# Runki2018/litehandnet

Measured on AMD Instinct MI355X. Metric: images/sec fwd+bwd @256x256 bs64 litehandnet, higher is better.
Workload: dtype f32; 1 GPU; litehandnet variant B (MSRB hourglass litehourglass.py) C=128, 256x256x3 -> 21x64x64, per-GPU batch 64, train-mode BN, fwd + TopdownHeatmapLoss + bwd + fused Adam; global_batch=64, parallelism=dp1

## Files before the change

### litehandnet_amd/csrc/k_conv_dw.hip

```cpp
#include <stdlib.h>
#include "lhn_common.h"

template <int K>
__global__ void __launch_bounds__(256) k_dw_fwd(lhn_view x, const float* __restrict__ w, lhn_view y,
                                                double* __restrict__ stats, int stride, int pad, int dil, lhn_bnfin fin,
                                                int ) {
  extern __shared__ __attribute__((aligned(16))) float smem[];
  const int C = x.C, C4 = C >> 2;
  constexpr int KK = K * K;
  float* Ws = smem;
  f4* red = reinterpret_cast<f4*>(smem + KK * C);
  const int tid = threadIdx.x;
  const int c4 = tid % C4, pl = tid / C4, PL = 256 / C4;
  const int cin = x.coff + 4 * c4, cout = y.coff + 4 * c4;
  const Xf4 xf = lhn_load_xf(x, cin);
  for (int i = tid; i < KK * C; i += 256) {
    const int c = i / KK, t = i - c * KK;
    Ws[t * C + c] = w ? w[i] : 1.f;
  }
  __syncthreads();
  f4 wt[KK];
#pragma unroll
  for (int t = 0; t < KK; ++t) wt[t] = *reinterpret_cast<const f4*>(Ws + t * C + 4 * c4);
  const int rows = y.N * y.H;
// ... 1064 lines not shown
        const int ih = h0 + ph, iw = w0 + pw;
        const bool inb = ih >= 0 && ih < SH && iw >= 0 && iw < SW;
        f4 v = lhn_apply_xf(raw[it], xf) * gate;
        if (NS > 1) {
          v += lhn_apply_xf(raw2[it], xf2) * gate2;
          if (ex.sum_out && cok && inb && ph >= T::P && ph < T::P + TH && pw >= T::P && pw < T::P + TW)
            *reinterpret_cast<f4*>(ex.sum_out + ((size_t)(n * x.H + pa + ps * ih) * x.W + pb + ps * iw) * ex.so_cstride + ex.so_coff +
                                   cg * 32 + 4 * c4) = v;
        }
        tile[i * 8 + c4] = inb ? v : (f4){0.f, 0.f, 0.f, 0.f};
      }
    }
    __syncthreads();
    if (t + (int)gridDim.x < ntile) issue(t + gridDim.x);
    const int wo = tw * TW + pl;
    f4 s = (f4){0.f, 0.f, 0.f, 0.f}, q = s, kk = s;
    int cnt = 0;
    if (wo < SW && cok) {
      const f4* col = tile + (pl + T::P) * 8 + c4;
      float* yout = y.data + ((size_t)(n * y.H + pa + ps * th * TH) * y.W + pb + ps * wo) * y.cstride + cout;
      if (K == 3 && DIL == 1) {
        f4 wt[9];
#pragma unroll
        for (int k = 0; k < 9; ++k) wt[k] = wl[k * 8 + c4];
        f4 win[3][3];
#pragma unroll
        for (int a = 0; a < 2; ++a)
#pragma unroll
          for (int b = 0; b < 3; ++b) win[a + 1][b] = col[(a * T::WW + (b - 1)) * 8];
#pragma unroll
        for (int rr = 0; rr < TH; ++rr) {
#pragma unroll
          for (int b = 0; b < 3; ++b) {
            win[0][b] = win[1][b];
            win[1][b] = win[2][b];
            win[2][b] = col[((rr + 2) * T::WW + (b - 1)) * 8];
          }
          if (th * TH + rr < SH) {
            f4 acc = (f4){0.f, 0.f, 0.f, 0.f};
#pragma unroll
            for (int a = 0; a < 3; ++a)
#pragma unroll
              for (int b = 0; b < 3; ++b) acc += win[a][b] * wt[a * 3 + b];
            *reinterpret_cast<f4*>(yout + (size_t)rr * ps * y.W * y.cstride) = acc;
            if (cnt == 0) kk = acc;
            const f4 d = acc - kk;
            s += d;
            q += d * d;
            ++cnt;
          }
        }
      } else {
        for (int rr = 0; rr < TH; ++rr) {
          if (th * TH + rr >= SH) break;
          f4 acc = (f4){0.f, 0.f, 0.f, 0.f};
#pragma unroll
          for (int a = 0; a < K; ++a)
#pragma unroll
            for (int b = 0; b < K; ++b)
              acc += col[((rr + a * DIL) * T::WW + (b * DIL - T::P)) * 8] * wl[(a * K + b) * 8 + c4];
          *reinterpret_cast<f4*>(yout + (size_t)rr * ps * y.W * y.cstride) = acc;
          if (cnt == 0) kk = acc;
          const f4 d = acc - kk;
          s += d;
          q += d * d;
          ++cnt;
        }
      }
    }
    lhn_unshift4(sd, qd, s, q, kk, cnt);
  }
  if (stats) {
    const int C = x.C;
    double* st = stats + (size_t)((bid / cgroups) % LHN_STAT_REPLICAS) * 2 * C + cg * 32;
    lhn_block_stat_atomics_d(sd, qd, 8, reinterpret_cast<double*>(red), st, st + C, cvalid);
    if (fin.counter && lhn_last_block(fin.counter)) lhn_bn_finalize_block_par(fin, stats, reinterpret_cast<double*>(red));
  }
}

struct DwBnSum {
  double* sums;
  const float* save;
  int C, coff;
  const float* add[2];
};

template <int K, int DIL, bool BNS = false>
__global__ void __launch_bounds__(256) k_dwk_bwd_lds(lhn_view x, const float* __restrict__ w, lhn_view y, lhn_gradview gy,
                                                     float* __restrict__ dx, int dx_acc, float* __restrict__ dw, int tiles_h,
                                                     int tiles_w, int cgroups, int nrep, int64_t rep_stride, int ps, DwBnSum bs, int xchunk) {
  constexpr int TH = 8, TW = 16, KK = K * K;
  const int bid = xchunk ? (int)(blockIdx.x & 7) * xchunk + (int)(blockIdx.x >> 3) : (int)blockIdx.x;
  constexpr bool REGACC = (K == 3);
  using T = DwTile<K, DIL, TH, TW>;
  extern __shared__ __attribute__((aligned(16))) float smem[];
  f4* tdy = reinterpret_cast<f4*>(smem);
  f4* tx = tdy + T::PIX * 8;
  f4* red = tx + T::PIX * 8;
  f4* wl = red + 256;
  f4* dws = wl + KK * 8;
  f4* traw = dws + KK * 8;
  f4* tmi = traw + TH * TW * 8;
  const int tid = threadIdx.x, c4 = tid & 7, pl = tid >> 3;
  const int colw = pl & 15, rpar = pl >> 4;
  const int ntile = y.N * ps * ps * tiles_h * tiles_w * cgroups;
  const int cg = bid % cgroups;
  const int cvalid = min(8, (x.C - cg * 32) >> 2);
  const bool cok = c4 < cvalid;
  const int c4e = cok ? c4 : 0;
  const int cx = x.coff + cg * 32 + 4 * c4e, cy = y.coff + cg * 32 + 4 * c4e;
  const Xf4 xxf = lhn_load_xf(x, cx), yxf = lhn_load_xf(y, cy);
  const Gr4 ygr = lhn_load_coef(gy, y.cstride, cy);
  for (int i = tid; i < KK * 8; i += 256) {
    const int k = i >> 3, cc = cg * 32 + 4 * min(i & 7, cvalid - 1);
    wl[i] = (f4){w[(cc + 0) * KK + k], w[(cc + 1) * KK + k], w[(cc + 2) * KK + k], w[(cc + 3) * KK + k]};
    if (!REGACC) dws[i] = (f4){0.f, 0.f, 0.f, 0.f};
  }
  f4 accw[REGACC ? KK : 1];
#pragma unroll
  for (int k = 0; k < (REGACC ? KK : 1); ++k) accw[k] = (f4){0.f, 0.f, 0.f, 0.f};
  f4 sdu = (f4){0.f, 0.f, 0.f, 0.f}, sdux = sdu;
  if (BNS && tid < 16) {
    const int kind = tid >> 3, cc = tid & 7;
    tmi[tid] = *reinterpret_cast<const f4*>(bs.save + kind * bs.C + bs.coff + cg * 32 + 4 * cc);
  }
  for (int t = bid; t < ntile; t += gridDim.x) {
    int r = t / cgroups;
    const int tw = r % tiles_w;
    r /= tiles_w;
    const int th = r % tiles_h;
    r /= tiles_h;
    const int par = r % (ps * ps), n = r / (ps * ps), pa = par / ps, pb = par % ps;
    const int SH = (x.H - pa + ps - 1) / ps, SW = (x.W - pb + ps - 1) / ps;
    const f4 xgate = x.gate ? *reinterpret_cast<const f4*>(x.gate + (size_t)n * x.cstride + cx) : (f4){1.f, 1.f, 1.f, 1.f};
    const f4 ygate = y.gate ? *reinterpret_cast<const f4*>(y.gate + (size_t)n * y.cstride + cy) : (f4){1.f, 1.f, 1.f, 1.f};
    const int h0 = th * TH - T::P, w0 = tw * TW - T::P;
    __syncthreads();
    {
      constexpr int NIT = (T::PIX + 31) / 32;
      f4 rx[NIT], ry[NIT], rz[NIT];
#pragma unroll
      for (int it = 0; it < NIT; ++it) {
        const int i = min(pl + 32 * it, T::PIX - 1);
        const int ph = i / T::WW, pw = i - ph * T::WW;
        const int ih = min(pa + ps * min(max(h0 + ph, 0), max(SH - 1, 0)), x.H - 1);
        const int iw = min(pb + ps * min(max(w0 + pw, 0), max(SW - 1, 0)), x.W - 1);
        const size_t pix = (size_t)(n * x.H + ih) * x.W + iw;
        rx[it] = *reinterpret_cast<const f4*>(x.data + pix * x.cstride + cx);
        ry[it] = *reinterpret_cast<const f4*>(y.data + pix * y.cstride + cy);
        rz[it] = *reinterpret_cast<const f4*>(gy.dz + pix * y.cstride + cy);
      }
#pragma unroll
      for (int it = 0; it < NIT; ++it) {
        const int i = pl + 32 * it;
        if (i < T::PIX) {
          const int ph = i / T::WW, pw = i - ph * T::WW;
          const int ih = h0 + ph, iw = w0 + pw;
          const bool inb = ih >= 0 && ih < SH && iw >= 0 && iw < SW;
          const f4 vx = lhn_apply_xf(rx[it], xxf) * xgate;
          f4 e = rz[it] * ygate;
          const f4 u = ry[it] * yxf.sc + yxf.sh;
          const f4 dl = (f4){u.x > 0.f ? 1.f : yxf.sl.x, u.y > 0.f ? 1.f : yxf.sl.y, u.z > 0.f ? 1.f : yxf.sl.z,
                             u.w > 0.f ? 1.f : yxf.sl.w};
          if (gy.dpool && inb) e += lhn_dpool_sum(gy, y, n, pa + ps * ih, pb + ps * iw, cy);
          const f4 vy = ygr.A * (e * dl) + ygr.B * ry[it] + ygr.Cc;
          const f4 z = (f4){0.f, 0.f, 0.f, 0.f};
          tx[i * 8 + c4] = inb ? vx : z;
          tdy[i * 8 + c4] = inb ? vy : z;
          if (BNS && ph >= T::P && ph < T::P + TH && pw >= T::P && pw < T::P + TW) traw[((ph - T::P) * TW + pw - T::P) * 8 + c4] = rx[it];
        }
      }
    }
    __syncthreads();
    const int wcol = tw * TW + colw;
    if (REGACC) {
#pragma unroll
      for (int j = 0; j < TH / 2; ++j) {
        const int rr = 2 * j + rpar, hh = th * TH + rr;
        if (wcol < SW && hh < SH) {
          const int centre = ((rr + T::P) * T::WW + colw + T::P) * 8 + c4;
          const f4 dyc = tdy[centre];
          f4 accx = (f4){0.f, 0.f, 0.f, 0.f};
#pragma unroll
          for (int a = 0; a < K; ++a)
#pragma unroll
            for (int b = 0; b < K; ++b) {
              const int off = ((a * DIL - T::P) * T::WW + (b * DIL - T::P)) * 8;
              accx += tdy[centre - off] * wl[(a * K + b) * 8 + c4];
              accw[REGACC ? a * K + b : 0] += dyc * tx[centre + off];
            }
          if (BNS) {
            const f4 raw = traw[(rr * TW + colw) * 8 + c4];
            const f4 u = raw * xxf.sc + xxf.sh;
            const f4 du = accx * (f4){u.x > 0.f ? 1.f : xxf.sl.x, u.y > 0.f ? 1.f : xxf.sl.y, u.z > 0.f ? 1.f : xxf.sl.z, u.w > 0.f ? 1.f : xxf.sl.w};
            sdu += du;
            sdux += du * ((raw - tmi[c4]) * tmi[8 + c4]);
          }
          if (dx && cok) {
            float* o = dx + ((size_t)(n * x.H + pa + ps * hh) * x.W + pb + ps * wcol) * x.cstride + cx;
            if (dx_acc) accx += *reinterpret_cast<const f4*>(o);
            if (bs.add[0]) accx += *reinterpret_cast<const f4*>(bs.add[0] + (o - dx));
            if (bs.add[1]) accx += *reinterpret_cast<const f4*>(bs.add[1] + (o - dx));
            *reinterpret_cast<f4*>(o) = accx;
          }
        }
      }
    } else {
      if (dx)
        for (int j = 0; j < TH / 2; ++j) {
          const int rr = 2 * j + rpar, hh = th * TH + rr;
          if (wcol < SW && hh < SH && cok) {
            const int centre = ((rr + T::P) * T::WW + colw + T::P) * 8 + c4;
            f4 accx = (f4){0.f, 0.f, 0.f, 0.f};
            for (int a = 0; a < K; ++a)
#pragma unroll
              for (int b = 0; b < K; ++b)
                accx += tdy[centre - ((a * DIL - T::P) * T::WW + (b * DIL - T::P)) * 8] * wl[(a * K + b) * 8 + c4];
            float* o = dx + ((size_t)(n * x.H + pa + ps * hh) * x.W + pb + ps * wcol) * x.cstride + cx;
            if (dx_acc) accx += *reinterpret_cast<const f4*>(o);
            if (bs.add[0]) accx += *reinterpret_cast<const f4*>(bs.add[0] + (o - dx));
            if (bs.add[1]) accx += *reinterpret_cast<const f4*>(bs.add[1] + (o - dx));
            *reinterpret_cast<f4*>(o) = accx;
          }
        }
      for (int a = 0; a < K; ++a) {
        f4 ar[K];
#pragma unroll
        for (int b = 0; b < K; ++b) ar[b] = (f4){0.f, 0.f, 0.f, 0.f};
        for (int j = 0; j < TH / 2; ++j) {
          const int rr = 2 * j + rpar, hh = th * TH + rr;
          if (wcol < SW && hh < SH) {
            const int centre = ((rr + T::P) * T::WW + colw + T::P) * 8 + c4;
            const f4 dyc = tdy[centre];
#pragma unroll
            for (int b = 0; b < K; ++b) ar[b] += dyc * tx[centre + ((a * DIL - T::P) * T::WW + (b * DIL - T::P)) * 8];
          }
        }
#pragma unroll
        for (int b = 0; b < K; ++b) {
          f4 v = ar[b];
#pragma unroll
          for (int o = 8; o < 64; o <<= 1) {
            v.x += __shfl_xor(v.x, o, 64);
            v.y += __shfl_xor(v.y, o, 64);
            v.z += __shfl_xor(v.z, o, 64);
            v.w += __shfl_xor(v.w, o, 64);
          }
          if ((tid & 63) < 8) red[(tid >> 6) * 8 + c4 + 32 * b] = v;
        }
        __syncthreads();
        if (tid < 8 * K) {
          const int b = tid >> 3, cc = tid & 7;
          dws[(a * K + b) * 8 + cc] += red[cc + 32 * b] + red[8 + cc + 32 * b] + red[16 + cc + 32 * b] + red[24 + cc + 32 * b];
        }
        __syncthreads();
      }
    }
  }
  if (BNS) {
    double* st = bs.sums + (size_t)((bid / cgroups) % LHN_STAT_REPLICAS) * 2 * bs.C + bs.coff + cg * 32;
    lhn_block_stat_atomics(sdu, sdux, 8, red, st, st + bs.C);
  }
  float* dwr = dw + (size_t)((bid / cgroups) % nrep) * rep_stride;
  if (REGACC) {
#pragma unroll
    for (int k = 0; k < KK; ++k)
#pragma unroll
      for (int o = 8; o < 64; o <<= 1) {
        accw[k].x += __shfl_xor(accw[k].x, o, 64);
        accw[k].y += __shfl_xor(accw[k].y, o, 64);
        accw[k].z += __shfl_xor(accw[k].z, o, 64);
        accw[k].w += __shfl_xor(accw[k].w, o, 64);
      }
    __syncthreads();
    if ((tid & 63) < 8)
#pragma unroll
      for (int k = 0; k < KK; ++k) tdy[(k * 4 + (tid >> 6)) * 8 + c4] = accw[k];
    __syncthreads();
    if (tid < KK * 8) {
      const int k = tid >> 3, cc = tid & 7;
      const f4 sacc = tdy[(k * 4 + 0) * 8 + cc] + tdy[(k * 4 + 1) * 8 + cc] + tdy[(k * 4 + 2) * 8 + cc] + tdy[(k * 4 + 3) * 8 + cc];
      const int cb = cg * 32 + 4 * cc;
      if (cc < cvalid) {
        atomicAdd(dwr + (cb + 0) * KK + k, sacc.x);
        atomicAdd(dwr + (cb + 1) * KK + k, sacc.y);
        atomicAdd(dwr + (cb + 2) * KK + k, sacc.z);
        atomicAdd(dwr + (cb + 3) * KK + k, sacc.w);
      }
    }
  } else {
    __syncthreads();
    for (int i = tid; i < KK * 8; i += 256) {
      const int k = i >> 3, cb = cg * 32 + 4 * (i & 7);
      const f4 v = dws[i];
      if ((i & 7) >= cvalid) continue;
      atomicAdd(dwr + (cb + 0) * KK + k, v.x);
      atomicAdd(dwr + (cb + 1) * KK + k, v.y);
      atomicAdd(dwr + (cb + 2) * KK + k, v.z);
      atomicAdd(dwr + (cb + 3) * KK + k, v.w);
    }
  }
}

static int dw3_xchunk(int grid, int cgroups) {
  static int on = -1;
  if (on < 0) {
    const char* e = getenv("LHN_XCD_ORDER");
    on = (e && e[0] == '1') ? 1 : 0;
  }
  return (on && grid % (8 * cgroups) == 0) ? grid / 8 : 0;
}
static int dw3_grid(int ntile, int cgroups, int per_cu) {
  int g = lhn_num_cus() * per_cu;
  g -= g % cgroups;
  if (g > ntile) g = ntile;
  if (g < cgroups) g = cgroups;
  return g;
}

template <int K, int DIL, int NS = 1>
static void launch_dwk_fwd(const lhn_view* x, const float* w, const lhn_view* y, double* stats, lhn_bnfin fin, hipStream_t s, int ps = 1,
                           const DwExtra* exp = nullptr) {
  DwExtra ex;
  if (exp) ex = *exp; else { ex.n = 0; ex.sum_out = nullptr; }
  constexpr int TH = 8, TW = 32, P = DIL * (K - 1) / 2;
  const int cg = (x->C + 31) / 32;
  const int sh = (y->H + ps - 1) / ps, sw = (y->W + ps - 1) / ps;
  const int th = (sh + TH - 1) / TH, tw = (sw + TW - 1) / TW, ntile = y->N * ps * ps * th * tw * cg;
  const size_t lds = (size_t)((TH + 2 * P) * (TW + 2 * P) * 8 + 512 + K * K * 8) * 16;
  const int per_cu = lds > 80 * 1024 ? 1 : (lds > 52 * 1024 ? 2 : 3);
  static LhnKernelCfg cfg;
  (void)lhn_kernel_cfg(cfg, &k_dwk_fwd_lds<K, DIL, NS>, lds, 4, nullptr);
  const int grid = dw3_grid(ntile, cg, per_cu * 2);
  hipLaunchKernelGGL((k_dwk_fwd_lds<K, DIL, NS>), dim3(grid), dim3(256), lds, s, *x, w, *y, stats, th, tw, cg, fin, ps, ex, dw3_xchunk(grid, cg));
}
template <int K, int DIL, bool BNS = false>
static void launch_dwk_bwd(const lhn_view* x, const float* w, const lhn_view* y, const lhn_gradview* gy, float* dx, int dx_acc,
                           float* dw, int nrep, int64_t rep_stride, hipStream_t s, int ps = 1, const DwBnSum* bsp = nullptr) {
  constexpr int TH = 8, TW = 16, P = DIL * (K - 1) / 2;
  DwBnSum bs;
  if (bsp) bs = *bsp; else { bs.sums = nullptr; bs.save = nullptr; bs.C = bs.coff = 0; bs.add[0] = bs.add[1] = nullptr; }
  const int cg = (x->C + 31) / 32;
  const int sh = (x->H + ps - 1) / ps, sw = (x->W + ps - 1) / ps;
  const int th = (sh + TH - 1) / TH, tw = (sw + TW - 1) / TW, ntile = x->N * ps * ps * th * tw * cg;
  const size_t lds = (size_t)((TH + 2 * P) * (TW + 2 * P) * 16 + 256 + 2 * K * K * 8 + (BNS ? TH * TW * 8 + 16 : 0)) * 16;
  static LhnKernelCfg cfg;
  (void)lhn_kernel_cfg(cfg, &k_dwk_bwd_lds<K, DIL, BNS>, lds, 4, nullptr);
  const int grid = dw3_grid(ntile, cg, 4);
  hipLaunchKernelGGL((k_dwk_bwd_lds<K, DIL, BNS>), dim3(grid), dim3(256), lds, s, *x, w, *y, *gy, dx, dx_acc, dw, th, tw,
                     cg, nrep, rep_stride, ps, bs, dw3_xchunk(grid, cg));
}


struct DwS2 {
  static constexpr int TH = 4, TW = 16, XH = 2 * TH + 1, XW = 2 * TW + 1, XPIX = XH * XW, DH = TH + 1, DW = TW + 1, DPIX = DH * DW;
};

__global__ void __launch_bounds__(256) k_dws2_fwd_lds(lhn_view x, const float* __restrict__ w, lhn_view y, double* __restrict__ stats,
                                                      int tiles_h, int tiles_w, int cgroups, lhn_bnfin fin) {
  using T = DwS2;
  extern __shared__ __attribute__((aligned(16))) float smem[];
  f4* tx = reinterpret_cast<f4*>(smem);
  f4* red = tx + T::XPIX * 8;
  f4* wl = red + 512;
  const int tid = threadIdx.x, c4 = tid & 7, pl = tid >> 3;
  const int ntile = y.N * tiles_h * tiles_w * cgroups;
  const int cg = blockIdx.x % cgroups;
  const int cvalid = min(8, (x.C - cg * 32) >> 2);
  const bool cok = c4 < cvalid;
  const int c4e = cok ? c4 : 0;
  const int cin = x.coff + cg * 32 + 4 * c4e, cout = y.coff + cg * 32 + 4 * c4e;
  for (int i = tid; i < 72; i += 256) {
    const int k = i >> 3, cc = cg * 32 + 4 * min(i & 7, cvalid - 1);
    wl[i] = (f4){w[(cc + 0) * 9 + k], w[(cc + 1) * 9 + k], w[(cc + 2) * 9 + k], w[(cc + 3) * 9 + k]};
  }
  const Xf4 xf = lhn_load_xf(x, cin);
  double sd[4] = {0, 0, 0, 0}, qd[4] = {0, 0, 0, 0};
  constexpr int NIT = (T::XPIX + 31) / 32;
  for (int t = blockIdx.x; t < ntile; t += gridDim.x) {
    int r = t / cgroups;
    const int tw = r % tiles_w;
    r /= tiles_w;
    const int th = r % tiles_h, n = r / tiles_h;
    const int h0 = 2 * th * T::TH - 1, w0 = 2 * tw * T::TW - 1;
    const f4 gate = x.gate ? *reinterpret_cast<const f4*>(x.gate + (size_t)n * x.cstride + cin) : (f4){1.f, 1.f, 1.f, 1.f};
    const float* xin = x.data + (size_t)n * x.H * x.W * x.cstride + cin;
    f4 raw[NIT];
#pragma unroll
    for (int it = 0; it < NIT; ++it) {
      const int i = min(pl + 32 * it, T::XPIX - 1);
      const int ph = i / T::XW, pw = i - ph * T::XW;
      const int ih = min(max(h0 + ph, 0), x.H - 1), iw = min(max(w0 + pw, 0), x.W - 1);
      raw[it] = *reinterpret_cast<const f4*>(xin + ((size_t)ih * x.W + iw) * x.cstride);
    }
    __syncthreads();
#pragma unroll
    for (int it = 0; it < NIT; ++it) {
      const int i = pl + 32 * it;
      if (i < T::XPIX) {
        const int ph = i / T::XW, pw = i - ph * T::XW;
        const int ih = h0 + ph, iw = w0 + pw;
        const bool inb = ih >= 0 && ih < x.H && iw >= 0 && iw < x.W;
        tx[i * 8 + c4] = inb ? lhn_apply_xf(raw[it], xf) * gate : (f4){0.f, 0.f, 0.f, 0.f};
      }
    }
    __syncthreads();
    f4 s = (f4){0.f, 0.f, 0.f, 0.f}, q = s, kk = s;
    int cnt = 0;
#pragma unroll
    for (int j = 0; j < 2; ++j) {
      const int o = pl + 32 * j, oh = o / T::TW, ow = o - oh * T::TW;
      const int ho = th * T::TH + oh, wo = tw * T::TW + ow;
      if (cok && ho < y.H && wo < y.W) {
        f4 acc = (f4){0.f, 0.f, 0.f, 0.f};
#pragma unroll
        for (int a = 0; a < 3; ++a)
#pragma unroll
          for (int b = 0; b < 3; ++b) acc += tx[((2 * oh + a) * T::XW + 2 * ow + b) * 8 + c4] * wl[(a * 3 + b) * 8 + c4];
        *reinterpret_cast<f4*>(y.data + ((size_t)(n * y.H + ho) * y.W + wo) * y.cstride + cout) = acc;
        if (cnt == 0) kk = acc;
        const f4 d = acc - kk;
        s += d;
        q += d * d;
        ++cnt;
      }
    }
    lhn_unshift4(sd, qd, s, q, kk, cnt);
  }
  if (stats) {
    const int C = x.C;
    double* st = stats + (size_t)((blockIdx.x / cgroups) % LHN_STAT_REPLICAS) * 2 * C + cg * 32;
    lhn_block_stat_atomics_d(sd, qd, 8, reinterpret_cast<double*>(red), st, st + C, cvalid);
    if (fin.counter && lhn_last_block(fin.counter)) lhn_bn_finalize_block(fin, stats);
  }
}

__global__ void __launch_bounds__(256, 2) k_dws2_bwd_lds(lhn_view x, const float* __restrict__ w, lhn_view y, lhn_gradview gy,
                                                      float* __restrict__ dx, int dx_acc, float* __restrict__ dw, int tiles_h,
                                                      int tiles_w, int cgroups, int nrep, int64_t rep_stride) {
  using T = DwS2;
  extern __shared__ __attribute__((aligned(16))) float smem[];
  f4* tx = reinterpret_cast<f4*>(smem);
  f4* tdy = tx + T::XPIX * 8;
  f4* wl = tdy + T::DPIX * 8;
  const int tid = threadIdx.x, c4 = tid & 7, pl = tid >> 3;
  const int ntile = y.N * tiles_h * tiles_w * cgroups;
  const int cg = blockIdx.x % cgroups;
  const int cvalid = min(8, (x.C - cg * 32) >> 2);
  const bool cok = c4 < cvalid;
  const int c4e = cok ? c4 : 0;
  const int cx = x.coff + cg * 32 + 4 * c4e, cy = y.coff + cg * 32 + 4 * c4e;
  const Xf4 xxf = lhn_load_xf(x, cx), yxf = lhn_load_xf(y, cy);
  const Gr4 ygr = lhn_load_coef(gy, y.cstride, cy);
  for (int i = tid; i < 72; i += 256) {
    const int k = i >> 3, cc = cg * 32 + 4 * min(i & 7, cvalid - 1);
    wl[i] = (f4){w[(cc + 0) * 9 + k], w[(cc + 1) * 9 + k], w[(cc + 2) * 9 + k], w[(cc + 3) * 9 + k]};
  }
  f4 accw[9];
#pragma unroll
  for (int k = 0; k < 9; ++k) accw[k] = (f4){0.f, 0.f, 0.f, 0.f};
  constexpr int NITX = (T::XPIX + 31) / 32, NITD = (T::DPIX + 31) / 32;
  for (int t = blockIdx.x; t < ntile; t += gridDim.x) {
    int r = t / cgroups;
    const int tw = r % tiles_w;
    r /= tiles_w;
    const int th = r % tiles_h, n = r / tiles_h;
    const int h0 = 2 * th * T::TH - 1, w0 = 2 * tw * T::TW - 1;
    const int oh0 = th * T::TH, ow0 = tw * T::TW;
    const f4 xgate = x.gate ? *reinterpret_cast<const f4*>(x.gate + (size_t)n * x.cstride + cx) : (f4){1.f, 1.f, 1.f, 1.f};
    f4 rx[NITX], ry[NITD], rz[NITD];
#pragma unroll
    for (int it = 0; it < NITX; ++it) {
      const int i = min(pl + 32 * it, T::XPIX - 1);
      const int ph = i / T::XW, pw = i - ph * T::XW;
      const int ih = min(max(h0 + ph, 0), x.H - 1), iw = min(max(w0 + pw, 0), x.W - 1);
      rx[it] = *reinterpret_cast<const f4*>(x.data + ((size_t)(n * x.H + ih) * x.W + iw) * x.cstride + cx);
    }
#pragma unroll
    for (int it = 0; it < NITD; ++it) {
      const int i = min(pl + 32 * it, T::DPIX - 1);
      const int ph = i / T::DW, pw = i - ph * T::DW;
      const int ho = min(oh0 + ph, y.H - 1), wo = min(ow0 + pw, y.W - 1);
      const size_t off = ((size_t)(n * y.H + ho) * y.W + wo) * y.cstride + cy;
      ry[it] = *reinterpret_cast<const f4*>(y.data + off);
      rz[it] = *reinterpret_cast<const f4*>(gy.dz + off);
    }
    __syncthreads();
#pragma unroll
    for (int it = 0; it < NITX; ++it) {
      const int i = pl + 32 * it;
      if (i < T::XPIX) {
        const int ph = i / T::XW, pw = i - ph * T::XW;
        const int ih = h0 + ph, iw = w0 + pw;
        const bool inb = ih >= 0 && ih < x.H && iw >= 0 && iw < x.W;
        tx[i * 8 + c4] = inb ? lhn_apply_xf(rx[it], xxf) * xgate : (f4){0.f, 0.f, 0.f, 0.f};
      }
    }
#pragma unroll
    for (int it = 0; it < NITD; ++it) {
      const int i = pl + 32 * it;
      if (i < T::DPIX) {
        const int ph = i / T::DW, pw = i - ph * T::DW;
        const int ho = oh0 + ph, wo = ow0 + pw;
        f4 d = (f4){0.f, 0.f, 0.f, 0.f};
        if (ho < y.H && wo < y.W) {
          const f4 du = lhn_grad_du(y, gy, yxf, ry[it], rz[it], n, ho, wo, cy);
          d = ygr.A * du + ygr.B * ry[it] + ygr.Cc;
        }
        tdy[i * 8 + c4] = d;
      }
    }
    __syncthreads();
#pragma unroll
    for (int j = 0; j < 2; ++j) {
      const int o = pl + 32 * j, oh = o / T::TW, ow = o - oh * T::TW;
      const f4 dyc = tdy[(oh * T::DW + ow) * 8 + c4];
#pragma unroll
      for (int a = 0; a < 3; ++a)
#pragma unroll
        for (int b = 0; b < 3; ++b) accw[a * 3 + b] += dyc * tx[((2 * oh + a) * T::XW + 2 * ow + b) * 8 + c4];
    }
    if (dx && cok) {
      const int c = pl, iw = 2 * ow0 + c;
      const int nb = (c & 1) ? 2 : 1;
      const int bA = (c & 1) ? 0 : 1, colA = (c & 1) ? (c + 1) >> 1 : c >> 1, colB = (c - 1) >> 1;
      if (iw < x.W) {
#pragma unroll
        for (int rr = 0; rr < 2 * T::TH; ++rr) {
          const int ih = 2 * oh0 + rr;
          if (ih < x.H) {
            f4 accx = (f4){0.f, 0.f, 0.f, 0.f};
            if ((rr & 1) == 0) {
              const f4* drow = tdy + ((rr >> 1) * T::DW) * 8 + c4;
              accx += drow[colA * 8] * wl[(3 + bA) * 8 + c4];
              if (nb == 2) accx += drow[colB * 8] * wl[(3 + 2) * 8 + c4];
            } else {
              const f4* d0 = tdy + (((rr + 1) >> 1) * T::DW) * 8 + c4;
              const f4* d2 = tdy + (((rr - 1) >> 1) * T::DW) * 8 + c4;
              accx += d0[colA * 8] * wl[(0 + bA) * 8 + c4] + d2[colA * 8] * wl[(6 + bA) * 8 + c4];
              if (nb == 2) accx += d0[colB * 8] * wl[(0 + 2) * 8 + c4] + d2[colB * 8] * wl[(6 + 2) * 8 + c4];
            }
            float* o = dx + ((size_t)(n * x.H + ih) * x.W + iw) * x.cstride + cx;
            if (dx_acc) accx += *reinterpret_cast<const f4*>(o);
            *reinterpret_cast<f4*>(o) = accx;
          }
        }
      }
    }
  }
  float* dwr = dw + (size_t)((blockIdx.x / cgroups) % nrep) * rep_stride;
#pragma unroll
  for (int k = 0; k < 9; ++k)
#pragma unroll
    for (int o = 8; o < 64; o <<= 1) {
      accw[k].x += __shfl_xor(accw[k].x, o, 64);
      accw[k].y += __shfl_xor(accw[k].y, o, 64);
      accw[k].z += __shfl_xor(accw[k].z, o, 64);
      accw[k].w += __shfl_xor(accw[k].w, o, 64);
    }
  __syncthreads();
  if ((tid & 63) < 8)
#pragma unroll
    for (int k = 0; k < 9; ++k) tdy[(k * 4 + (tid >> 6)) * 8 + c4] = accw[k];
  __syncthreads();
  if (tid < 72) {
    const int k = tid >> 3, cc = tid & 7;
    const f4 sacc = tdy[(k * 4 + 0) * 8 + cc] + tdy[(k * 4 + 1) * 8 + cc] + tdy[(k * 4 + 2) * 8 + cc] + tdy[(k * 4 + 3) * 8 + cc];
    const int cb = cg * 32 + 4 * cc;
    if (cc < cvalid) {
      atomicAdd(dwr + (cb + 0) * 9 + k, sacc.x);
      atomicAdd(dwr + (cb + 1) * 9 + k, sacc.y);
      atomicAdd(dwr + (cb + 2) * 9 + k, sacc.z);
      atomicAdd(dwr + (cb + 3) * 9 + k, sacc.w);
    }
  }
}

static int dws2_fwd(const lhn_view* x, const float* w, const lhn_view* y, double* stats, lhn_bnfin fin, hipStream_t s) {
  using T = DwS2;
  const int cg = (x->C + 31) / 32;
  const int th = (y->H + T::TH - 1) / T::TH, tw = (y->W + T::TW - 1) / T::TW, ntile = y->N * th * tw * cg;
  size_t lds = (size_t)(T::XPIX * 8 + 512 + 72) * 16;
  static LhnKernelCfg cfg;
  if (!lhn_kernel_cfg(cfg, &k_dws2_fwd_lds, lds, 4, nullptr)) return 0;
  hipLaunchKernelGGL(k_dws2_fwd_lds, dim3(dw3_grid(ntile, cg, 6)), dim3(256), lds, s, *x, w, *y, stats, th, tw, cg, fin);
  return 1;
}
static int dws2_bwd(const lhn_view* x, const float* w, const lhn_view* y, const lhn_gradview* gy, float* dx, int dx_acc, float* dw,
                    int nrep, int64_t rep_stride, hipStream_t s) {
  using T = DwS2;
  const int cg = (x->C + 31) / 32;
  const int th = (y->H + T::TH - 1) / T::TH, tw = (y->W + T::TW - 1) / T::TW, ntile = y->N * th * tw * cg;
  const size_t lds = (size_t)((T::XPIX + T::DPIX) * 8 + 72) * 16;
  static LhnKernelCfg cfg;
  if (!lhn_kernel_cfg(cfg, &k_dws2_bwd_lds, lds, 4, nullptr)) return 0;
  hipLaunchKernelGGL(k_dws2_bwd_lds, dim3(dw3_grid(ntile, cg, 4)), dim3(256), lds, s, *x, w, *y, *gy, dx, dx_acc, dw, th, tw, cg, nrep, rep_stride);
  return 1;
}

int lhn_dwk_fwd_lds(const lhn_view* x, const float* w, const lhn_view* y, double* stats, int k, int dil, lhn_bnfin fin,
                    hipStream_t s, const DwExtra* ex) {
  if (ex && ex->n > 0) {
    if (k == 3 && dil == 1) launch_dwk_fwd<3, 1, 2>(x, w, y, stats, fin, s, 1, ex);
    else if (k == 3 && dil == 2 && y->W >= 16) launch_dwk_fwd<3, 1, 2>(x, w, y, stats, fin, s, 2, ex);
    else return 0;
    return 1;
  }
  if (k == 3 && dil == 1) launch_dwk_fwd<3, 1>(x, w, y, stats, fin, s, 1, ex);
  else if (k == 3 && dil == 2 && y->W >= 16) launch_dwk_fwd<3, 1>(x, w, y, stats, fin, s, 2, ex);
  else if (k == 3 && dil == 2) launch_dwk_fwd<3, 2>(x, w, y, stats, fin, s, 1, ex);
  else if (k == 7 && dil == 1) launch_dwk_fwd<7, 1>(x, w, y, stats, fin, s, 1, ex);
  else return 0;
  return 1;
}
int lhn_dwk_bwd_lds(const lhn_view* x, const float* w, const lhn_view* y, const lhn_gradview* gy, float* dx, int dx_acc,
                    float* dw, int k, int dil, int nrep, int64_t rep_stride, hipStream_t s, const DwBnSum* bs) {
  if (bs && bs->sums) {
    if (!(k == 3 && dil == 1 && dx && !dx_acc)) return 0;
    launch_dwk_bwd<3, 1, true>(x, w, y, gy, dx, dx_acc, dw, nrep, rep_stride, s, 1, bs);
    return 1;
  }
  if (k == 3 && dil == 1) launch_dwk_bwd<3, 1>(x, w, y, gy, dx, dx_acc, dw, nrep, rep_stride, s, 1, bs);
  else if (k == 3 && dil == 2 && x->W >= 16) launch_dwk_bwd<3, 1>(x, w, y, gy, dx, dx_acc, dw, nrep, rep_stride, s, 2, bs);
  else if (k == 3 && dil == 2) launch_dwk_bwd<3, 2>(x, w, y, gy, dx, dx_acc, dw, nrep, rep_stride, s, 1, bs);
  else if (k == 7 && dil == 1) launch_dwk_bwd<7, 1>(x, w, y, gy, dx, dx_acc, dw, nrep, rep_stride, s, 1, bs);
  else return 0;
  return 1;
}

static int dw_fwd_extra(const lhn_view* x, const float* w, const lhn_view* y, double* stats, int k, int stride, int pad, int dil,
                        lhn_bnfin fin, const lhn_view* extra, const float* coef, const lhn_view* so, hipStream_t s) {
  if (!(stride == 1 && pad == dil * (k - 1) / 2 && x->C % 4 == 0 && y->W >= 8)) return 0;
  if (!lhn_no_pend(x) || !lhn_no_pend(extra)) return 0;
  DwExtra ex;
  ex.v = *extra;
  ex.coef[0] = coef[0];
  ex.coef[1] = coef[1];
  ex.n = 1;
  ex.sum_out = so ? so->data : nullptr;
  ex.so_cstride = so ? so->cstride : 0;
  ex.so_coff = so ? so->coff : 0;
  return lhn_dwk_fwd_lds(x, w, y, stats, k, dil, fin, s, &ex);
}

static int dw_bwd_addends(const lhn_view* x, const float* w, const lhn_view* y, const lhn_gradview* gy, float* dx, int dx_acc, float* dw,
                          int k, int dil, int nrep, int64_t rep_stride, const float* a0, const float* a1, hipStream_t s) {
  DwBnSum bs;
  bs.sums = nullptr;
  bs.save = nullptr;
  bs.C = bs.coff = 0;
  bs.add[0] = a0;
  bs.add[1] = a1;
  return lhn_dwk_bwd_lds(x, w, y, gy, dx, dx_acc, dw, k, dil, nrep, rep_stride, s, &bs);
}

static int dw_bwd_fused(const lhn_view* x, const float* w, const lhn_view* y, const lhn_gradview* gy, float* dx, float* dw, int k,
                        int dil, int nrep, int64_t rep_stride, double* bn_sums, const float* bn_save, int bn_C, int bn_coff, hipStream_t s) {
  DwBnSum bs;
  bs.sums = bn_sums;
  bs.save = bn_save;
  bs.C = bn_C;
  bs.coff = bn_coff;
  bs.add[0] = bs.add[1] = nullptr;
  return lhn_dwk_bwd_lds(x, w, y, gy, dx, 0, dw, k, dil, nrep, rep_stride, s, &bs);
}
```

Measured before the change: 8040 images/s.

## Add row-streaming depthwise 3x3 backward kernel with register prefetch and rolling LDS window

Adds a new depthwise 3x3 backward kernel that streams each 32-column strip down a chunk of rows. It keeps a small rolling ring of rows in LDS and prefetches the next row (or the next tile's first row) into registers while computing the current one. This replaces the 2D-tile backward for 3x3 kernels, including the BN-stat fused and dilated variants, and the old path stays reachable through an environment variable. The aim is to cut halo reloads and LDS footprint so occupancy goes up and global-load latency overlaps with compute. The cost is more complex indexing and a row-serial loop with a barrier per row.

Result: faster. 8240 images/s (median of 6 runs) (+2.5%).

```diff
diff --git a/litehandnet_amd/csrc/k_conv_dw.hip b/litehandnet_amd/csrc/k_conv_dw.hip
--- a/litehandnet_amd/csrc/k_conv_dw.hip
+++ b/litehandnet_amd/csrc/k_conv_dw.hip
@@ -1390,6 +1390,196 @@
   }
 }
 
+template <int DIL, bool BNS = false>
+__global__ void __launch_bounds__(256, (BNS || DIL > 1) ? 2 : 3) k_dw3_bwd_rows(lhn_view x, const float* __restrict__ w, lhn_view y, lhn_gradview gy,
+                                                         float* __restrict__ dx, int dx_acc, float* __restrict__ dw, int nstrips,
+                                                         int nchunks, int CH, int cgroups, int nrep, int64_t rep_stride, int ps,
+                                                         DwBnSum bs) {
+  constexpr int P = DIL, R = 2 * P + 2, WW = 32 + 2 * P, KK = 9;
+  extern __shared__ __attribute__((aligned(16))) float smem[];
+  f4* tdy = reinterpret_cast<f4*>(smem);
+  f4* tx = tdy + R * WW * 8;
+  f4* wl = tx + R * WW * 8;
+  f4* cst = wl + KK * 8;
+  f4* tmi = cst + KK * 8;
+  f4* traw = tmi + 16;
+  const int tid = threadIdx.x, c4 = tid & 7, pl = tid >> 3;
+  const int ntile = y.N * ps * ps * nchunks * nstrips * cgroups;
+  const int cg = blockIdx.x % cgroups;
+  const int cvalid = min(8, (x.C - cg * 32) >> 2);
+  const bool cok = c4 < cvalid;
+  const int c4e = cok ? c4 : 0;
+  const int cx = x.coff + cg * 32 + 4 * c4e, cy = y.coff + cg * 32 + 4 * c4e;
+  const bool edge = tid < 16 * P;
+  const int ecol = (pl < P) ? pl : 32 + pl;
+  const f4 z = (f4){0.f, 0.f, 0.f, 0.f}, one = (f4){1.f, 1.f, 1.f, 1.f};
+  if (tid < KK * 8) {
+    const int k = tid >> 3, cc = cg * 32 + 4 * min(tid & 7, cvalid - 1);
+    wl[tid] = (f4){w[(cc + 0) * KK + k], w[(cc + 1) * KK + k], w[(cc + 2) * KK + k], w[(cc + 3) * KK + k]};
+  } else if (tid < 2 * KK * 8) {
+    const int i = tid - KK * 8, kind = i >> 3, ca = cg * 32 + 4 * min(i & 7, cvalid - 1), j = kind % 3;
+    const float* tab = kind < 3 ? x.table : kind < 6 ? y.table : gy.coef;
+    const int cs = kind < 3 ? x.cstride : y.cstride, co = kind < 3 ? x.coff : y.coff;
+    cst[i] = tab ? *reinterpret_cast<const f4*>(tab + j * cs + co + ca) : ((kind < 6 ? j != 1 : j == 0) ? one : z);
+  } else if (BNS && tid < 2 * KK * 8 + 16) {
+    const int i = tid - 2 * KK * 8, kind = i >> 3, cc = i & 7;
+    tmi[i] = *reinterpret_cast<const f4*>(bs.save + kind * bs.C + bs.coff + cg * 32 + 4 * cc);
+  }
+  f4 accw[KK];
+#pragma unroll
+  for (int k = 0; k < KK; ++k) accw[k] = z;
+  f4 sdu = z, sdux = z;
+  struct Item {
+    int n, pa, pb, SH, SW, wb, h0, nrows;
+  };
+  auto decode = [&](int t) __attribute__((always_inline)) {
+    Item it;
+    int r = t / cgroups;
+    const int st = r % nstrips;
+    r /= nstrips;
+    const int ch = r % nchunks;
+    r /= nchunks;
+    const int par = r % (ps * ps);
+    it.n = r / (ps * ps);
+    it.pa = par / ps;
+    it.pb = par % ps;
+    it.SH = (x.H - it.pa + ps - 1) / ps;
+    it.SW = (x.W - it.pb + ps - 1) / ps;
+    it.wb = st * 32;
+    it.h0 = ch * CH;
+    it.nrows = max(0, min(CH, it.SH - it.h0));
+    return it;
+  };
+  f4 mx = z, my = z, mz = z, mp = z, ex = z, ey = z, ez = z, ep = z;
+  bool okm = false, oke = false;
+  auto issue = [&](const Item& it, int hr) __attribute__((always_inline)) {
+    const bool rok = hr >= 0 && hr < it.SH && cok;
+    const int ih = it.pa + ps * hr;
+    const int cm = it.wb + pl, ce = it.wb - P + ecol;
+    okm = rok && cm < it.SW;
+    oke = rok && edge && ce >= 0 && ce < it.SW;
+    mx = my = mz = mp = ex = ey = ez = ep = z;
+    if (okm) {
+      const size_t pix = (size_t)(it.n * x.H + ih) * x.W + it.pb + ps * cm;
+      mx = *reinterpret_cast<const f4*>(x.data + pix * x.cstride + cx);
+      my = *reinterpret_cast<const f4*>(y.data + pix * y.cstride + cy);
+      mz = *reinterpret_cast<const f4*>(gy.dz + pix * y.cstride + cy);
+      if (gy.dpool) mp = lhn_dpool_sum(gy, y, it.n, ih, it.pb + ps * cm, cy);
+    }
+    if (oke) {
+      const size_t pix = (size_t)(it.n * x.H + ih) * x.W + it.pb + ps * ce;
+      ex = *reinterpret_cast<const f4*>(x.data + pix * x.cstride + cx);
+      ey = *reinterpret_cast<const f4*>(y.data + pix * y.cstride + cy);
+      ez = *reinterpret_cast<const f4*>(gy.dz + pix * y.cstride + cy);
+      if (gy.dpool) ep = lhn_dpool_sum(gy, y, it.n, ih, it.pb + ps * ce, cy);
+    }
+  };
+  auto put = [&](int s, int col, bool ok, f4 rx, f4 ry, f4 rz, f4 rp, f4 xg, f4 yg) __attribute__((always_inline)) {
+    const f4 xsc = cst[c4], xsh = cst[8 + c4], xsl = cst[16 + c4];
+    const f4 ysc = cst[24 + c4], ysh = cst[32 + c4], ysl = cst[40 + c4];
+    const f4 gA = cst[48 + c4], gB = cst[56 + c4], gC = cst[64 + c4];
+    const f4 ux = rx * xsc + xsh;
+    const f4 vx = (f4){lhn_lrelu(ux.x, xsl.x), lhn_lrelu(ux.y, xsl.y), lhn_lrelu(ux.z, xsl.z), lhn_lrelu(ux.w, xsl.w)} * xg;
+    const f4 e = rz * yg + rp;
+    const f4 u = ry * ysc + ysh;
+    const f4 dl = (f4){u.x > 0.f ? 1.f : ysl.x, u.y > 0.f ? 1.f : ysl.y, u.z > 0.f ? 1.f : ysl.z, u.w > 0.f ? 1.f : ysl.w};
+    const f4 vy = gA * (e * dl) + gB * ry + gC;
+    tx[(s * WW + col) * 8 + c4] = ok ? vx : z;
+    tdy[(s * WW + col) * 8 + c4] = ok ? vy : z;
+    if (BNS && col >= P && col < 32 + P) traw[(s * 32 + col - P) * 8 + c4] = rx;
+  };
+  int t = blockIdx.x;
+  if (t < ntile) {
+    const Item nx = decode(t);
+    issue(nx, nx.h0 - P);
+  }
+#pragma unroll 1
+  for (; t < ntile; t += gridDim.x) {
+    const Item it = decode(t);
+    const f4 xg = x.gate ? *reinterpret_cast<const f4*>(x.gate + (size_t)it.n * x.cstride + cx) : one;
+    const f4 yg = y.gate ? *reinterpret_cast<const f4*>(y.gate + (size_t)it.n * y.cstride + cy) : one;
+    const int wcol = it.wb + pl, nload = it.nrows + 2 * P;
+    const bool ocol = wcol < it.SW;
+    __syncthreads();
+#pragma unroll 1
+    for (int q = 0; q < nload; ++q) {
+      const bool orow = q >= 2 * P;
+      const int hh = it.h0 + max(q - 2 * P, 0);
+      float* o = dx + ((size_t)(it.n * x.H + it.pa + ps * hh) * x.W + it.pb + ps * wcol) * x.cstride + cx;
+      const bool st = orow && dx && cok && ocol;
+      const int s = q % R;
+      put(s, pl + P, okm, mx, my, mz, mp, xg, yg);
+      if (edge) put(s, ecol, oke, ex, ey, ez, ep, xg, yg);
+      if (q + 1 < nload) issue(it, it.h0 - P + q + 1);
+      else if (t + (int)gridDim.x < ntile) {
+        const Item nx = decode(t + gridDim.x);
+        issue(nx, nx.h0 - P);
+      }
+      __syncthreads();
+      if (!orow || !ocol) continue;
+      int sr[3];
+#pragma unroll
+      for (int a = 0; a < 3; ++a) sr[a] = (q - 2 * P + a * DIL) % R;
+      const int centre = (sr[1] * WW + pl + P) * 8 + c4;
+      const f4 dyc = tdy[centre];
+      f4 accx = z;
+#pragma unroll
+      for (int a = 0; a < 3; ++a) {
+#pragma unroll
+        for (int b = 0; b < 3; ++b) {
+          accx += tdy[(sr[2 - a] * WW + pl + 2 * P - b * DIL) * 8 + c4] * wl[(a * 3 + b) * 8 + c4];
+          accw[a * 3 + b] += dyc * tx[(sr[a] * WW + pl + b * DIL) * 8 + c4];
+        }
+      }
+      if (BNS) {
+        const f4 raw = traw[(sr[1] * 32 + pl) * 8 + c4];
+        const f4 xsc = cst[c4], xsh = cst[8 + c4], xsl = cst[16 + c4];
+        const f4 u = raw * xsc + xsh;
+        const f4 du = accx * (f4){u.x > 0.f ? 1.f : xsl.x, u.y > 0.f ? 1.f : xsl.y, u.z > 0.f ? 1.f : xsl.z, u.w > 0.f ? 1.f : xsl.w};
+        sdu += du;
+        sdux += du * ((raw - tmi[c4]) * tmi[8 + c4]);
+      }
+      if (st) {
+        if (dx_acc) accx += *reinterpret_cast<const f4*>(o);
+        if (bs.add[0]) accx += *reinterpret_cast<const f4*>(bs.add[0] + (o - dx));
+        if (bs.add[1]) accx += *reinterpret_cast<const f4*>(bs.add[1] + (o - dx));
+        *reinterpret_cast<f4*>(o) = accx;
+      }
+    }
+  }
+  f4* red = tdy;
+  if (BNS) {
+    double* sts = bs.sums + (size_t)((blockIdx.x / cgroups) % LHN_STAT_REPLICAS) * 2 * bs.C + bs.coff + cg * 32;
+    lhn_block_stat_atomics(sdu, sdux, 8, red, sts, sts + bs.C);
+  }
+  float* dwr = dw + (size_t)((blockIdx.x / cgroups) % nrep) * rep_stride;
+#pragma unroll
+  for (int k = 0; k < KK; ++k)
+#pragma unroll
+    for (int o = 8; o < 64; o <<= 1) {
+      accw[k].x += __shfl_xor(accw[k].x, o, 64);
+      accw[k].y += __shfl_xor(accw[k].y, o, 64);
+      accw[k].z += __shfl_xor(accw[k].z, o, 64);
+      accw[k].w += __shfl_xor(accw[k].w, o, 64);
+    }
+  __syncthreads();
+  if ((tid & 63) < 8)
+#pragma unroll
+    for (int k = 0; k < KK; ++k) red[(k * 4 + (tid >> 6)) * 8 + c4] = accw[k];
+  __syncthreads();
+  if (tid < KK * 8) {
+    const int k = tid >> 3, cc = tid & 7;
+    const f4 sacc = red[(k * 4 + 0) * 8 + cc] + red[(k * 4 + 1) * 8 + cc] + red[(k * 4 + 2) * 8 + cc] + red[(k * 4 + 3) * 8 + cc];
+    const int cb = cg * 32 + 4 * cc;
+    if (cc < cvalid) {
+      atomicAdd(dwr + (cb + 0) * KK + k, sacc.x);
+      atomicAdd(dwr + (cb + 1) * KK + k, sacc.y);
+      atomicAdd(dwr + (cb + 2) * KK + k, sacc.z);
+      atomicAdd(dwr + (cb + 3) * KK + k, sacc.w);
+    }
+  }
+}
+
 static int dw3_xchunk(int grid, int cgroups) {
   static int on = -1;
   if (on < 0) {
@@ -1437,6 +1627,37 @@
   const int grid = dw3_grid(ntile, cg, 4);
   hipLaunchKernelGGL((k_dwk_bwd_lds<K, DIL, BNS>), dim3(grid), dim3(256), lds, s, *x, w, *y, *gy, dx, dx_acc, dw, th, tw,
                      cg, nrep, rep_stride, ps, bs, dw3_xchunk(grid, cg));
+}
+template <int DIL, bool BNS = false>
+static void launch_dw3_bwd_rows(const lhn_view* x, const float* w, const lhn_view* y, const lhn_gradview* gy, float* dx, int dx_acc,
+                                float* dw, int nrep, int64_t rep_stride, hipStream_t s, int ps = 1, const DwBnSum* bsp = nullptr) {
+  constexpr int P = DIL, R = 2 * P + 2, WW = 32 + 2 * P;
+  DwBnSum bs;
+  if (bsp) bs = *bsp; else { bs.sums = nullptr; bs.save = nullptr; bs.C = bs.coff = 0; bs.add[0] = bs.add[1] = nullptr; }
+  const int cg = (x->C + 31) / 32;
+  const int sh = (x->H + ps - 1) / ps, sw = (x->W + ps - 1) / ps;
+  const int nstrips = (sw + 31) / 32;
+  const size_t lds = (size_t)(2 * R * WW * 8 + 2 * 9 * 8 + 16 + (BNS ? R * 32 * 8 : 0)) * 16;
+  static LhnKernelCfg cfg;
+  int per_cu = 1;
+  (void)lhn_kernel_cfg(cfg, &k_dw3_bwd_rows<DIL, BNS>, lds, 8, &per_cu);
+  const int base = x->N * ps * ps * nstrips * cg;
+  int nch = (lhn_num_cus() * per_cu + base - 1) / base;
+  nch = std::max(1, std::min(nch, (sh + 7) / 8));
+  const int CH = (sh + nch - 1) / nch;
+  nch = (sh + CH - 1) / CH;
+  const int ntile = base * nch;
+  const int grid = dw3_grid(ntile, cg, per_cu);
+  hipLaunchKernelGGL((k_dw3_bwd_rows<DIL, BNS>), dim3(grid), dim3(256), lds, s, *x, w, *y, *gy, dx, dx_acc, dw, nstrips, nch, CH, cg,
+                     nrep, rep_stride, ps, bs);
+}
+static bool lhn_dw_bwd_v1() {
+  static int v = -1;
+  if (v < 0) {
+    const char* e = getenv("LHN_DW_BWD_V1");
+    v = (e && e[0] == '1') ? 1 : 0;
+  }
+  return v == 1;
 }
 
 
@@ -1705,13 +1926,21 @@
                     float* dw, int k, int dil, int nrep, int64_t rep_stride, hipStream_t s, const DwBnSum* bs) {
   if (bs && bs->sums) {
     if (!(k == 3 && dil == 1 && dx && !dx_acc)) return 0;
-    launch_dwk_bwd<3, 1, true>(x, w, y, gy, dx, dx_acc, dw, nrep, rep_stride, s, 1, bs);
+    if (lhn_dw_bwd_v1()) launch_dwk_bwd<3, 1, true>(x, w, y, gy, dx, dx_acc, dw, nrep, rep_stride, s, 1, bs);
+    else launch_dw3_bwd_rows<1, true>(x, w, y, gy, dx, dx_acc, dw, nrep, rep_stride, s, 1, bs);
     return 1;
   }
-  if (k == 3 && dil == 1) launch_dwk_bwd<3, 1>(x, w, y, gy, dx, dx_acc, dw, nrep, rep_stride, s, 1, bs);
-  else if (k == 3 && dil == 2 && x->W >= 16) launch_dwk_bwd<3, 1>(x, w, y, gy, dx, dx_acc, dw, nrep, rep_stride, s, 2, bs);
-  else if (k == 3 && dil == 2) launch_dwk_bwd<3, 2>(x, w, y, gy, dx, dx_acc, dw, nrep, rep_stride, s, 1, bs);
-  else if (k == 7 && dil == 1) launch_dwk_bwd<7, 1>(x, w, y, gy, dx, dx_acc, dw, nrep, rep_stride, s, 1, bs);
+  const bool v1 = lhn_dw_bwd_v1();
+  if (k == 3 && dil == 1) {
+    if (v1) launch_dwk_bwd<3, 1>(x, w, y, gy, dx, dx_acc, dw, nrep, rep_stride, s, 1, bs);
+    else launch_dw3_bwd_rows<1>(x, w, y, gy, dx, dx_acc, dw, nrep, rep_stride, s, 1, bs);
+  } else if (k == 3 && dil == 2 && x->W >= 16) {
+    if (v1) launch_dwk_bwd<3, 1>(x, w, y, gy, dx, dx_acc, dw, nrep, rep_stride, s, 2, bs);
+    else launch_dw3_bwd_rows<1>(x, w, y, gy, dx, dx_acc, dw, nrep, rep_stride, s, 2, bs);
+  } else if (k == 3 && dil == 2) {
+    if (v1) launch_dwk_bwd<3, 2>(x, w, y, gy, dx, dx_acc, dw, nrep, rep_stride, s, 1, bs);
+    else launch_dw3_bwd_rows<2>(x, w, y, gy, dx, dx_acc, dw, nrep, rep_stride, s, 1, bs);
+  } else if (k == 7 && dil == 1) launch_dwk_bwd<7, 1>(x, w, y, gy, dx, dx_acc, dw, nrep, rep_stride, s, 1, bs);
   else return 0;
   return 1;
 }
```
